# KhutornoyYaroslav/vcm-ts

Hardware: AMD Instinct MI355X
Metric: encoded frames/sec at 1920x1080 GOP-32 (higher is better)
Workload: dtype f32 (fp16x3 split-MFMA, fp32 accumulate)

## Files before the change

### vcm_ts_amd/csrc/conv_mfma.hip

```cpp
#include <hip/hip_runtime.h>
#include <stdint.h>
#include <stdlib.h>
#include <string.h>
#include <type_traits>
#include <vector>

#include "dcvc_hip.h"
#include "kernel_common.h"

namespace {

constexpr int LDK = 20;


struct ConvK {
    const float *seg_ptr[DCVC_MAX_SEG];
    int seg_C[DCVC_MAX_SEG];
    int seg_cs[DCVC_MAX_SEG];
    int nseg;
    int Hin, Win, Hout, Wout;
    int in_act;
    float in_slope;
    const float *wpack;
    const float *bpack;
    int Cout, Cout_pad;
    float *out;
    int out_cs;
    int out_act;
    float out_slope;
    int ps;
    const float *res;
    int res_cs;
    const float *res_gate;
    const float *res2;
    int res2_cs;
    int vec_epi;
    int *status;
    float *chan_partial;
    int ntx;
    int ty0, nty;
    int band_rows;
};

int g_lookahead = 2;

inline long dev_env_long(const char *name, long dflt) {
    const char *dev = getenv("DCVC_DEV");
    if (!dev || strcmp(dev, "1") != 0) return dflt;
    const char *v = getenv(name);
    return v ? atol(v) : dflt;
}


template <int KS, int S, int RPW, int NT, bool SPLIT, bool PAIR = false, bool AHEAD = false>
__global__ __launch_bounds__(256, 2) void conv_mfma(const ConvK a) {
    static_assert(!PAIR || (KS == 7 && S == 1 && SPLIT), "tap pairing is built for the 7x7 split-fp16 layers");
    constexpr int BH = 4 * RPW, BW = 32, BN = 32 * NT;
    constexpr int PH = (BH - 1) * S + KS, PW = (BW - 1) * S + KS, PAD = KS / 2;
    constexpr int T = PAIR ? KS * 4 : KS * KS;
    constexpr int TPS = PAIR ? 4 : (KS == 3 && S == 1) ? 9 : KS;
    constexpr int NST = T / TPS;
    constexpr int EPI_LD = BN + 4;
    constexpr int LDS_MAIN = PH * PW * LDK + TPS * 4 * BN * 4, LDS_EPI = 4 * 32 * EPI_LD, LDS_RED = 4 * BN;
    __shared__ __attribute__((aligned(16))) float lds[LDS_MAIN > LDS_EPI + LDS_RED ? LDS_MAIN : LDS_EPI + LDS_RED];
    float *patch = lds;
    float *wl = lds + PH * PW * LDK;

    const int tid = threadIdx.x, lane = tid & 63, wave = tid >> 6;
    const int nbn = a.Cout_pad / BN;
    const int nb = blockIdx.x % nbn, tx = blockIdx.x / nbn;
    if (tx >= a.ntx) return;
    const int ty = blockIdx.y + a.ty0;
    const int x0 = tx * BW, y0 = ty * BH, n0 = nb * BN, img = blockIdx.z;

    f32x16 acc[RPW][NT];
#pragma unroll
    for (int m = 0; m < RPW; ++m)
#pragma unroll
        for (int n = 0; n < NT; ++n)
#pragma unroll
            for (int r = 0; r < 16; ++r) acc[m][n][r] = 0.f;

    const int a_base = ((wave * RPW * S) * PW + (lane & 31) * S) * LDK + (lane >> 5) * 4;
    const int b_base = ((lane >> 5) * BN + (lane & 31)) * 4;

    constexpr int NP = (PH * PW * 4 + 255) / 256, NW = (TPS * 4 * BN + 255) / 256;
    static_assert(!AHEAD || NST >= 3, "AHEAD: two straight-line steps and a loop over the rest of a chunk");
    f32x4 rp[NP], rw[NW];
    struct Cursor {
        int s, c0, cg, st;
    };
    auto advance = [&](Cursor &k) {
        if (++k.st == NST) {
            k.st = 0;
            ++k.cg;
            k.c0 += MFMA_KC;
            if (k.c0 >= a.seg_C[k.s]) {
                ++k.s;
                k.c0 = 0;
            }
        }
    };
    int poff[NP];
    unsigned inpic = 0;
#pragma unroll
    for (int u = 0; u < NP; ++u) {
        const int i = tid + u * 256;
        const int p = i >> 2;
        const int py = p / PW, px = p - py * PW + (PAIR ? (i & 3) >> 1 : 0);
        const int gy = y0 * S - PAD + py, gx = x0 * S - PAD + px;
        const bool ok = i < PH * PW * 4 && gy >= 0 && gy < a.Hin && gx >= 0 && gx < a.Win;
        poff[u] = ok ? gy * a.Win + gx : 0;
        inpic |= (ok ? 1u : 0u) << u;
    }
    auto load_patch = [&](const Cursor &k) {
        const int C = a.seg_C[k.s], cs = a.seg_cs[k.s];
        const float *sp = a.seg_ptr[k.s] + (size_t)img * a.Hin * a.Win * cs;
        const int c = PAIR ? (tid & 1) * 4 : k.c0 + (tid & 3) * 4;
        const int cc = c < C ? c : 0;
#pragma unroll
        for (int u = 0; u < NP; ++u) rp[u] = *(const f32x4 *)(sp + (size_t)poff[u] * cs + cc);
    };
    auto store_patch = [&](const Cursor &k) {
        const int C = a.seg_C[k.s];
#pragma unroll
        for (int u = 0; u < NP; ++u) {
            const int i = tid + u * 256;
            if (i < PH * PW * 4) {
                const int c = PAIR ? (i & 1) * 4 : k.c0 + (i & 3) * 4;
                f32x4 v = ((inpic >> u) & 1u) && c < C ? rp[u] : (f32x4){0.f, 0.f, 0.f, 0.f};
                if (c + 3 >= C) {
                    if (c + 1 >= C) v[1] = 0.f;
                    if (c + 2 >= C) v[2] = 0.f;
                    v[3] = 0.f;
                }
                if (a.in_act) {
                    v[0] = act(v[0], a.in_slope);
                    v[1] = act(v[1], a.in_slope);
                    v[2] = act(v[2], a.in_slope);
                    v[3] = act(v[3], a.in_slope);
                }
                if (!SPLIT) {
                    *(f32x4 *)&patch[(i >> 2) * LDK + (i & 3) * 4] = v;
                } else {
                    f32x4 sv = v * ACT_SCALE;
#pragma unroll
                    for (int e = 0; e < 4; ++e) sv[e] = __builtin_amdgcn_fmed3f(sv[e], -F16_MAX, F16_MAX);
                    const f16x4 hi = __builtin_convertvector(sv, f16x4);
                    const f16x4 lo = __builtin_convertvector(sv - __builtin_convertvector(hi, f32x4), f16x4);
                    _Float16 *rec = (_Float16 *)&patch[(i >> 2) * LDK];
                    *(f16x4 *)&rec[(i & 3) * 4] = hi;
                    *(f16x4 *)&rec[16 + (i & 3) * 4] = lo;
                }
            }
        }
    };
    constexpr int W_OVER = NW * 256 - TPS * 4 * BN;
    static_assert(!AHEAD || TPS * 4 * BN >= W_OVER, "the doubled float4 must lie inside the slab");
    auto w_slot = [&](const int u) {
        const int i = tid + u * 256;
        return AHEAD && W_OVER > 0 && u == NW - 1 && i >= TPS * 4 * BN ? i - W_OVER : i;
    };
    auto load_w = [&](const Cursor &k) {
        const float *wsrc = a.wpack + ((size_t)(k.cg * T + k.st * TPS) * 4) * a.Cout_pad * 4 + (size_t)n0 * 4;
#pragma unroll
        for (int u = 0; u < NW; ++u) {
            const int i = w_slot(u);
            const int row = i / BN, col = i - row * BN;
            if (AHEAD || i < TPS * 4 * BN) rw[u] = *(const f32x4 *)(wsrc + ((size_t)row * a.Cout_pad + col) * 4);
        }
    };
    auto store_w = [&]() {
#pragma unroll
        for (int u = 0; u < NW; ++u) {
            const int i = w_slot(u);
            if (AHEAD || i < TPS * 4 * BN) *(f32x4 *)&wl[i * 4] = rw[u];
        }
    };
    auto mfma_step = [&](const int st) {
        const int a_st = (TPS == T) ? 0 : st * PW * LDK;
#pragma unroll
        for (int tt = 0; tt < TPS; ++tt) {
            const int ky = (TPS == T) ? tt / KS : 0, kx = PAIR ? 2 * tt : (TPS == T) ? tt % KS : tt;
            if (!SPLIT) {
#pragma unroll
                for (int k2 = 0; k2 < 2; ++k2) {
                    f32x4 af[RPW], bf[NT];
#pragma unroll
                    for (int m = 0; m < RPW; ++m)
                        af[m] = *(const f32x4 *)&patch[a_base + a_st + ((m * S + ky) * PW + kx) * LDK + k2 * 8];
#pragma unroll
                    for (int n = 0; n < NT; ++n)
                        bf[n] = *(const f32x4 *)&wl[b_base + ((tt * 4 + k2 * 2) * BN + n * 32) * 4];
#pragma unroll
                    for (int j = 0; j < 4; ++j)
#pragma unroll
                        for (int m = 0; m < RPW; ++m)
#pragma unroll
                            for (int n = 0; n < NT; ++n)
                                acc[m][n] = __builtin_amdgcn_mfma_f32_32x32x2f32(af[m][j], bf[n][j], acc[m][n], 0, 0, 0);
                }
            } else {
                f16x8 ah[RPW], al[RPW], bh[NT], bl[NT];
#pragma unroll
                for (int m = 0; m < RPW; ++m) {
                    const float *rec = &patch[a_base + a_st + ((m * S + ky) * PW + kx) * LDK];
                    ah[m] = *(const f16x8 *)rec;
                    al[m] = *(const f16x8 *)(rec + 8);
                }
#pragma unroll
                for (int n = 0; n < NT; ++n) {
                    bh[n] = *(const f16x8 *)&wl[b_base + ((tt * 4) * BN + n * 32) * 4];
                    bl[n] = *(const f16x8 *)&wl[b_base + ((tt * 4 + 2) * BN + n * 32) * 4];
                }
#pragma unroll
                for (int m = 0; m < RPW; ++m)
#pragma unroll
                    for (int n = 0; n < NT; ++n) {
                        acc[m][n] = __builtin_amdgcn_mfma_f32_32x32x16_f16(ah[m], bh[n], acc[m][n], 0, 0, 0);
                        acc[m][n] = __builtin_amdgcn_mfma_f32_32x32x16_f16(ah[m], bl[n], acc[m][n], 0, 0, 0);
                        acc[m][n] = __builtin_amdgcn_mfma_f32_32x32x16_f16(al[m], bh[n], acc[m][n], 0, 0, 0);
                    }
            }
        }
    };

    Cursor cur = {0, 0, 0, 0};
    if constexpr (AHEAD) {
        auto chunk = [&](auto more, const Cursor &nc) {
            constexpr bool MORE = decltype(more)::value;
            __syncthreads();
            store_patch(cur);
            store_w();
            __syncthreads();
            advance(cur);
            load_w(cur);
            if (MORE) load_patch(nc);
            mfma_step(0);
            auto row_step = [&](const int st) {
                __syncthreads();
                store_w();
                __syncthreads();
                if (st + 1 < NST) {
                    advance(cur);
                    load_w(cur);
                } else if (MORE) {
                    load_w(nc);
                }
                mfma_step(st);
            };
            row_step(1);
            for (int st = 2; st < NST; ++st) row_step(st);
        };
        load_patch(cur);
        load_w(cur);
        for (;;) {
            Cursor nc = cur;
            nc.st = NST - 1;
            advance(nc);
            if (nc.s >= a.nseg) break;
            chunk(std::true_type{}, nc);
            cur = nc;
        }
        chunk(std::false_type{}, cur);
    } else {
        load_patch(cur);
        load_w(cur);
        while (cur.s < a.nseg) {
            __syncthreads();
            if (cur.st == 0) store_patch(cur);
            store_w();
            __syncthreads();
            Cursor nxt = cur;
            advance(nxt);
            if (nxt.s < a.nseg) {
                if (nxt.st == 0) load_patch(nxt);
                load_w(nxt);
            }
            mfma_step(cur.st);
            cur = nxt;
        }
    }

    const int col = lane & 31, hh = lane >> 5;
    const int Cq = a.Cout >> 2;
    const int Cfin = a.ps ? Cq : a.Cout;
    const int Ho = a.ps ? a.Hout * 2 : a.Hout, Wo = a.ps ? a.Wout * 2 : a.Wout;
    const float inv_scale = SPLIT ? 1.f / (ACT_SCALE * WGT_SCALE) : 1.f;
    float vmax = 0.f;
    if (a.vec_epi) {
        constexpr int LPP = BN / 4, PPI = 64 / LPP, NIT = 32 / PPI;
        float *epi = lds + wave * 32 * EPI_LD;
        const int c4 = (lane % LPP) * 4, pl = lane / LPP;
        const int ch = n0 + c4;
        const bool ch_ok = ch < a.Cout;
        int dy = 0, dx = 0, cf = ch;
        if (a.ps) {
            const int sub = ch / Cq;
            cf = ch - sub * Cq;
            dy = sub >> 1;
            dx = sub & 1;
        }
        f32x4 bias = {0.f, 0.f, 0.f, 0.f}, gate = {1.f, 1.f, 1.f, 1.f};
        if (ch_ok) {
            bias = *(const f32x4 *)&a.bpack[ch];
            if (a.res_gate) gate = *(const f32x4 *)&a.res_gate[(size_t)img * Cfin + cf];
        }
        __syncthreads();
        size_t pix[RPW][NIT];
        bool ok[RPW][NIT];
        f32x4 rv[RPW][NIT], rv2[RPW][NIT];
        f32x4 csum = {0.f, 0.f, 0.f, 0.f};
#pragma unroll
        for (int m = 0; m < RPW; ++m) {
            const int oy = y0 + wave * RPW + m;
#pragma unroll
            for (int it = 0; it < NIT; ++it) {
                const int ox = x0 + it * PPI + pl;
                ok[m][it] = ch_ok && oy < a.Hout && ox < a.Wout;
                pix[m][it] = a.ps ? ((size_t)(img * Ho + 2 * oy + dy) * Wo + 2 * ox + dx) : ((size_t)(img * Ho + oy) * Wo + ox);
                rv[m][it] = (f32x4){0.f, 0.f, 0.f, 0.f};
                rv2[m][it] = (f32x4){0.f, 0.f, 0.f, 0.f};
                if (ok[m][it] && a.res) rv[m][it] = *(const f32x4 *)&a.res[pix[m][it] * a.res_cs + cf];
                if (ok[m][it] && a.res2) rv2[m][it] = *(const f32x4 *)&a.res2[pix[m][it] * a.res2_cs + cf];
            }
        }
#pragma unroll
        for (int m = 0; m < RPW; ++m) {
#pragma unroll
            for (int n = 0; n < NT; ++n)
#pragma unroll
                for (int r = 0; r < 16; ++r)
                    epi[((r & 3) + 8 * (r >> 2) + 4 * hh) * EPI_LD + n * 32 + col] = acc[m][n][r];
            asm volatile("s_waitcnt lgkmcnt(0)" ::: "memory");
#pragma unroll
            for (int it = 0; it < NIT; ++it) {
                f32x4 v = *(const f32x4 *)&epi[(it * PPI + pl) * EPI_LD + c4];
                v = v * inv_scale + bias;
                if (a.out_act == 1) {
                    v[0] = act(v[0], a.out_slope);
                    v[1] = act(v[1], a.out_slope);
                    v[2] = act(v[2], a.out_slope);
                    v[3] = act(v[3], a.out_slope);
                } else if (a.out_act == 2) {
#pragma unroll
                    for (int e = 0; e < 4; ++e) v[e] = fminf(fmaxf(v[e], 0.f), 1.f);
                }
                if (a.out_act == 3) {
#pragma unroll
                    for (int e = 0; e < 4; ++e) {
                        const float mk = rv2[m][it][e] > 0.f ? 1.f : a.out_slope;
                        v[e] = a.res ? __builtin_fmaf(v[e], mk, rv[m][it][e]) : v[e] * mk;
                    }
                } else {
                    if (a.res) {
                        if (a.res_gate) {
#pragma unroll
                            for (int e = 0; e < 4; ++e) v[e] = __builtin_fmaf(rv[m][it][e], gate[e], v[e]);
                        } else {
                            v = v + rv[m][it];
                        }
                    }
                    if (a.res2) v = rv2[m][it] + v;
                }
                if (a.chan_partial && ok[m][it]) csum += v;
                if (a.status && ok[m][it])
                    vmax = fmaxf(vmax, fmaxf(fmaxf(fabsf(v[0]), fabsf(v[1])), fmaxf(fabsf(v[2]), fabsf(v[3]))));
                if (ok[m][it]) *(f32x4 *)&a.out[pix[m][it] * a.out_cs + cf] = v;
            }
            asm volatile("s_waitcnt lgkmcnt(0)" ::: "memory");
        }
        if (a.status && !(vmax <= ACT_LIMIT)) atomicOr(a.status, DCVC_STATUS_ACT_SATURATED);
        if (a.chan_partial) {
#pragma unroll
            for (int off = LPP; off < 64; off <<= 1)
#pragma unroll
                for (int e = 0; e < 4; ++e) csum[e] += __shfl_xor(csum[e], off);
            float *red = lds + LDS_EPI;
            if (lane < LPP) *(f32x4 *)&red[wave * BN + c4] = csum;
            __syncthreads();
            if (tid < BN && n0 + tid < a.Cout_pad) {
                const float s = ((red[tid] + red[BN + tid]) + red[2 * BN + tid]) + red[3 * BN + tid];
                const size_t part = (size_t)img * (a.nty * a.ntx) + (size_t)ty * a.ntx + tx;
                a.chan_partial[part * a.Cout_pad + n0 + tid] = s;
            }
        }
        return;
    }
#pragma unroll
    for (int m = 0; m < RPW; ++m) {
        const int oy = y0 + wave * RPW + m;
        if (oy >= a.Hout) continue;
#pragma unroll
        for (int n = 0; n < NT; ++n) {
            const int ch = n0 + n * 32 + col;
            if (ch >= a.Cout) continue;
            const float bias = a.bpack[ch];
            int dy = 0, dx = 0, cf = ch;
            if (a.ps) {
                const int sub = ch / Cq;
                cf = ch - sub * Cq;
                dy = sub >> 1;
                dx = sub & 1;
            }
            const float gate = a.res_gate ? a.res_gate[(size_t)img * Cfin + cf] : 1.f;
            float rv[16], rv2[16];
#pragma unroll
            for (int r = 0; r < 16; ++r) {
                const int ox = x0 + (r & 3) + 8 * (r >> 2) + 4 * hh;
                const size_t pix = a.ps ? ((size_t)(img * Ho + 2 * oy + dy) * Wo + 2 * ox + dx)
                                        : ((size_t)(img * Ho + oy) * Wo + ox);
                rv[r] = (a.res && ox < a.Wout) ? a.res[pix * a.res_cs + cf] : 0.f;
                rv2[r] = (a.res2 && ox < a.Wout) ? a.res2[pix * a.res2_cs + cf] : 0.f;
            }
#pragma unroll
            for (int r = 0; r < 16; ++r) {
                const int ox = x0 + (r & 3) + 8 * (r >> 2) + 4 * hh;
                if (ox >= a.Wout) continue;
                float v = acc[m][n][r] * inv_scale + bias;
                if (a.out_act == 1) v = act(v, a.out_slope);
                else if (a.out_act == 2) v = fminf(fmaxf(v, 0.f), 1.f);
                const size_t pix = a.ps ? ((size_t)(img * Ho + 2 * oy + dy) * Wo + 2 * ox + dx)
                                        : ((size_t)(img * Ho + oy) * Wo + ox);
                if (a.out_act == 3) {
                    const float mk = rv2[r] > 0.f ? 1.f : a.out_slope;
                    v = a.res ? __builtin_fmaf(v, mk, rv[r]) : v * mk;
                } else {
                    if (a.res) v = a.res_gate ? __builtin_fmaf(rv[r], gate, v) : v + rv[r];
                    if (a.res2) v = rv2[r] + v;
                }
                if (a.status) vmax = fmaxf(vmax, fabsf(v));
                a.out[pix * a.out_cs + cf] = v;
            }
        }
    }
    if (a.status && !(vmax <= ACT_LIMIT)) atomicOr(a.status, DCVC_STATUS_ACT_SATURATED);
}


template <int KS, int S, int RPW, int NT, bool PAIR = false>
int launch(ConvK &k, int N, hipStream_t st, int precision) {
    constexpr int BH = 4 * RPW, BN = 32 * NT;
    k.ntx = (k.Wout + 31) / 32;
    static const bool xcd_pad = dev_env_long("DCVC_XCD_PAD", 0) != 0;
    unsigned gx = (unsigned)(k.ntx * (k.Cout_pad / BN));
    if (xcd_pad && gx >= 8) gx = (gx + 7) & ~7u;
    k.nty = (k.Hout + BH - 1) / BH;
    if (k.ty0 < 0 || k.ty0 >= k.nty) return DCVC_E_ARG;
    const int rows = k.band_rows > 0 ? (k.band_rows < k.nty - k.ty0 ? k.band_rows : k.nty - k.ty0) : k.nty;
    dim3 grid(gx, (unsigned)rows, (unsigned)N);
    constexpr bool HAS_AHEAD = (KS == 3 && S == 2) || KS == 7;
    if constexpr (HAS_AHEAD) {
        if (g_lookahead == 2) {
            if (PAIR)
                hipLaunchKernelGGL((conv_mfma<KS, S, RPW, NT, true, PAIR, true>), grid, dim3(256), 0, st, k);
            else if (precision == DCVC_PREC_FP16X3)
                hipLaunchKernelGGL((conv_mfma<KS, S, RPW, NT, true, false, true>), grid, dim3(256), 0, st, k);
            else
                hipLaunchKernelGGL((conv_mfma<KS, S, RPW, NT, false, false, !(KS == 7 && RPW == 2 && NT == 2)>), grid, dim3(256), 0, st, k);
            RET_LAUNCH();
        }
    }
    if (PAIR)
        hipLaunchKernelGGL((conv_mfma<KS, S, RPW, NT, true, PAIR>), grid, dim3(256), 0, st, k);
    else if (precision == DCVC_PREC_FP16X3)
        hipLaunchKernelGGL((conv_mfma<KS, S, RPW, NT, true>), grid, dim3(256), 0, st, k);
    else
        hipLaunchKernelGGL((conv_mfma<KS, S, RPW, NT, false>), grid, dim3(256), 0, st, k);
    RET_LAUNCH();
}

}

extern "C" int64_t dcvc_conv_pack_size(int32_t Cout, int32_t ks, int32_t nseg, const int32_t *seg_C, int32_t *cout_pad) {
    if (Cout <= 0 || nseg <= 0 || nseg > DCVC_MAX_SEG || (ks != 1 && ks != 3 && ks != 7)) return DCVC_E_ARG;
    int chunks = 0;
    for (int s = 0; s < nseg; ++s) chunks += (seg_C[s] + MFMA_KC - 1) / MFMA_KC;
    const int cp = round_up(Cout, 32);
    if (cout_pad) *cout_pad = cp;
    return (int64_t)chunks * ks * ks * 4 * cp * 4;
}

extern "C" int dcvc_conv_pack_weights(const float *w, const float *b, int32_t Cout, int32_t ks, int32_t nseg,
                                      const int32_t *seg_C, int32_t pixel_shuffle, int32_t precision, float *wpack,
                                      float *bpack) {
    if (precision != DCVC_PREC_FP32 && precision != DCVC_PREC_FP16X3) return DCVC_E_ARG;
    int32_t cp = 0;
    const int64_t total = dcvc_conv_pack_size(Cout, ks, nseg, seg_C, &cp);
    if (total < 0 || (pixel_shuffle && (Cout & 3))) return DCVC_E_ARG;
    const int T = ks * ks;
    int Cin = 0;
    for (int s = 0; s < nseg; ++s) Cin += seg_C[s];
    memset(wpack, 0, (size_t)total * sizeof(float));
    memset(bpack, 0, (size_t)cp * sizeof(float));
    const int Cq = Cout / 4;
    _Float16 *base = (_Float16 *)wpack;
    int cg = 0, cin0 = 0;
    for (int s = 0; s < nseg; ++s) {
        for (int c0 = 0; c0 < seg_C[s]; c0 += MFMA_KC, ++cg) {
            for (int t = 0; t < T; ++t)
                for (int cc = 0; cc < MFMA_KC && c0 + cc < seg_C[s]; ++cc)
                    for (int n = 0; n < Cout; ++n) {
                        const int np = pixel_shuffle ? ps_packed_channel(n, Cq) : n;
                        const float v = w[((size_t)n * Cin + cin0 + c0 + cc) * T + t];
                        if (precision == DCVC_PREC_FP32) {
                            wpack[mfma_wpack_f32(cg, T, t, cc, cp, np)] = v;
                        } else {
                            float sv = v * WGT_SCALE;
                            sv = sv > F16_MAX ? F16_MAX : (sv < -F16_MAX ? -F16_MAX : sv);
                            const SplitF16 p = split_f16(sv);
                            base[mfma_wpack_f16(cg, T, t, cc, cp, np, 0)] = p.hi;
                            base[mfma_wpack_f16(cg, T, t, cc, cp, np, 1)] = p.lo;
                        }
                    }
        }
        cin0 += seg_C[s];
    }
    for (int n = 0; n < Cout; ++n) bpack[pixel_shuffle ? ps_packed_channel(n, Cq) : n] = b ? b[n] : 0.f;
    return DCVC_OK;
}

extern "C" int64_t dcvc_conv_pack_size_paired(int32_t Cout, int32_t Cin, int32_t *cout_pad) {
    if (Cout <= 0 || Cin <= 0 || Cin > 8) return DCVC_E_ARG;
    const int cp = round_up(Cout, 32);
    if (cout_pad) *cout_pad = cp;
    return (int64_t)7 * 4 * 4 * cp * 4;
}

extern "C" int dcvc_conv_pack_weights_paired(const float *w, const float *b, int32_t Cout, int32_t Cin, float *wpack, float *bpack) {
    int32_t cp = 0;
    const int64_t total = dcvc_conv_pack_size_paired(Cout, Cin, &cp);
    if (total < 0 || !w || !wpack || !bpack) return DCVC_E_ARG;
    memset(wpack, 0, (size_t)total * sizeof(float));
    memset(bpack, 0, (size_t)cp * sizeof(float));
    _Float16 *base = (_Float16 *)wpack;
    bool clamped = false;
    for (int ky = 0; ky < 7; ++ky)
        for (int kx = 0; kx < 7; ++kx) {
            const int step = ky * 4 + (kx >> 1), h = kx & 1;
            for (int c = 0; c < Cin; ++c)
                for (int n = 0; n < Cout; ++n) {
                    float sv = w[((size_t)n * Cin + c) * 49 + ky * 7 + kx] * WGT_SCALE;
                    if (!(fabsf(sv) <= F16_MAX)) { clamped = true; sv = sv > 0.f ? F16_MAX : -F16_MAX; }
                    const SplitF16 p = split_f16(sv);
                    base[mfma_wpack_f16(0, 28, step, 8 * h + c, cp, n, 0)] = p.hi;
                    base[mfma_wpack_f16(0, 28, step, 8 * h + c, cp, n, 1)] = p.lo;
                }
        }
    for (int n = 0; n < Cout; ++n) bpack[n] = b ? b[n] : 0.f;
    return clamped ? DCVC_E_RANGE : DCVC_OK;
}

static int tile_rows(int ks, int stride) { return stride == 2 ? 4 : 8; }

extern "C" int32_t dcvc_conv_tile_rows(int32_t ks, int32_t stride) { return tile_rows(ks, stride); }

extern "C" int32_t dcvc_conv_chan_partial_parts(int32_t ks, int32_t stride, int32_t Hout, int32_t Wout) {
    if (Hout <= 0 || Wout <= 0 || (stride != 1 && stride != 2)) return DCVC_E_ARG;
    const int bh = tile_rows(ks, stride);
    return ((Wout + 31) / 32) * ((Hout + bh - 1) / bh);
}

extern "C" int dcvc_conv_set_lookahead(int32_t mode) {
    if (mode != 1 && mode != 2) return DCVC_E_ARG;
    g_lookahead = mode;
    return DCVC_OK;
}

extern "C" int dcvc_conv2d(const dcvc_conv_args *a, void *stream) {
    if (!conv_args_ok(a)) return DCVC_E_ARG;
    if (a->stride != 1 && a->stride != 2) return DCVC_E_ARG;
    if (a->precision != DCVC_PREC_FP32 && a->precision != DCVC_PREC_FP16X3) return DCVC_E_ARG;
    if (a->Cout_pad % 32 || a->Cout > a->Cout_pad || (a->pixel_shuffle && (a->Cout & 3))) return DCVC_E_ARG;
    if (a->out_act < 0 || a->out_act > 3) return DCVC_E_ARG;
    if (a->out_act == 3 && (!a->res2 || a->res_gate || a->chan_partial || a->pixel_shuffle)) return DCVC_E_ARG;
    ConvK k;
    memset(&k, 0, sizeof(k));
    copy_conv_args_full(k, a);
    k.Hin = a->Hin;
    k.Win = a->Win;
    const int pad = a->ks / 2;
    k.Hout = (a->Hin + 2 * pad - a->ks) / a->stride + 1;
    k.Wout = (a->Win + 2 * pad - a->ks) / a->stride + 1;
    k.vec_epi = vec_epilogue_ok(a);
    if (a->chan_partial && (!k.vec_epi || a->pixel_shuffle)) return DCVC_E_ARG;
    hipStream_t st = (hipStream_t)stream;
    const bool wide = (a->Cout_pad % 64) == 0;
    const int key = a->ks * 10 + a->stride;
    if (a->stride == 1 && !a->pair_taps && !a->chan_partial && a->tile_rows <= 0) {
        const long wgs8 = (long)((k.Wout + 31) / 32) * ((k.Hout + 7) / 8) * (a->Cout_pad / (wide ? 64 : 32)) * a->N;
        static const long rows4_below = dev_env_long("DCVC_ROWS4_WGS", 384);
        if (wgs8 < rows4_below) {
            if (a->ks == 3) return wide ? launch<3, 1, 1, 2>(k, a->N, st, a->precision) : launch<3, 1, 1, 1>(k, a->N, st, a->precision);
            if (a->ks == 7) return wide ? launch<7, 1, 1, 2>(k, a->N, st, a->precision) : launch<7, 1, 1, 1>(k, a->N, st, a->precision);
            if (a->ks == 1) return wide ? launch<1, 1, 1, 2>(k, a->N, st, a->precision) : launch<1, 1, 1, 1>(k, a->N, st, a->precision);
        }
    }
    switch (key) {
        case 11: return wide ? launch<1, 1, 2, 2>(k, a->N, st, a->precision) : launch<1, 1, 2, 1>(k, a->N, st, a->precision);
        case 12: return wide ? launch<1, 2, 1, 2>(k, a->N, st, a->precision) : launch<1, 2, 1, 1>(k, a->N, st, a->precision);
        case 31:
            return wide ? launch<3, 1, 2, 2>(k, a->N, st, a->precision) : launch<3, 1, 2, 1>(k, a->N, st, a->precision);
        case 32: return wide ? launch<3, 2, 1, 2>(k, a->N, st, a->precision) : launch<3, 2, 1, 1>(k, a->N, st, a->precision);
        case 71:
            if (a->pair_taps) {
                if (a->nseg != 1 || a->seg[0].C > 8 || a->precision != DCVC_PREC_FP16X3 || a->pixel_shuffle) return DCVC_E_ARG;
                return wide ? launch<7, 1, 2, 2, true>(k, a->N, st, a->precision) : launch<7, 1, 2, 1, true>(k, a->N, st, a->precision);
            }
            return wide ? launch<7, 1, 2, 2>(k, a->N, st, a->precision) : launch<7, 1, 2, 1>(k, a->N, st, a->precision);
        default: return DCVC_E_ARG;
    }
}
```

### vcm_ts_amd/csrc/conv_small.hip

```cpp
#include <hip/hip_runtime.h>
#include <stdint.h>
#include <string.h>

#include "dcvc_hip.h"
#include "kernel_common.h"

namespace {

constexpr int KC = 16;

struct SmallK {
    const float *seg_ptr[DCVC_MAX_SEG];
    int seg_C[DCVC_MAX_SEG];
    int seg_cs[DCVC_MAX_SEG];
    int nseg;
    int H, W;
    int in_act;
    float in_slope;
    const char *wpack;
    const float *bpack;
    int Cout;
    float *out;
    int out_cs, out_act;
    float out_slope;
    const float *res;
    int res_cs;
    int *status;
};

template <int KS>
__global__ __launch_bounds__(256, 3) void conv_small(const SmallK a) {
    constexpr int RPW = 2, BH = 4 * RPW, BW = 32, PAD = KS / 2, PH = BH + KS - 1, PW = BW + KS - 1, T = KS * KS;
    constexpr int TPS = KS, NST = KS;
    constexpr int PATCH_F = PH * PW * 16;
    constexpr int SLAB_F = TPS * 4 * 16 * 4;
    __shared__ __attribute__((aligned(16))) float lds[PATCH_F + SLAB_F];
    char *patch = (char *)lds;
    float *wl = lds + PATCH_F;

    const int tid = threadIdx.x, lane = tid & 63, wave = tid >> 6;
    const int x0 = blockIdx.x * BW, y0 = blockIdx.y * BH, img = blockIdx.z;
    const int pr = lane & 15, g = lane >> 4;

    f32x4 acc[RPW][2];
#pragma unroll
    for (int m = 0; m < RPW; ++m)
#pragma unroll
        for (int hf = 0; hf < 2; ++hf) acc[m][hf] = (f32x4){0.f, 0.f, 0.f, 0.f};

    constexpr int NP = (PH * PW * 4 + 255) / 256, NW = (SLAB_F / 4 + 255) / 256;
    f32x4 rp[NP], rw[NW];
    struct Cursor {
        int s, c0, cg, st;
    };
    auto advance = [&](Cursor &k) {
        if (++k.st == NST) {
            k.st = 0;
            ++k.cg;
            k.c0 += KC;
            if (k.c0 >= a.seg_C[k.s]) {
                ++k.s;
                k.c0 = 0;
            }
        }
    };
    int poff[NP];
    unsigned inpic = 0;
#pragma unroll
    for (int u = 0; u < NP; ++u) {
        const int i = tid + u * 256;
        const int p = i >> 2;
        const int py = p / PW, px = p - py * PW;
        const int gy = y0 - PAD + py, gx = x0 - PAD + px;
        const bool ok = i < PH * PW * 4 && gy >= 0 && gy < a.H && gx >= 0 && gx < a.W;
        poff[u] = ok ? gy * a.W + gx : 0;
        inpic |= (ok ? 1u : 0u) << u;
    }
    auto load_patch = [&](const Cursor &k) {
        const int C = a.seg_C[k.s], cs = a.seg_cs[k.s];
        const float *sp = a.seg_ptr[k.s] + (size_t)img * a.H * a.W * cs;
        const int c = k.c0 + (tid & 3) * 4;
        const int cc = c < C ? c : 0;
#pragma unroll
        for (int u = 0; u < NP; ++u) rp[u] = *(const f32x4 *)(sp + (size_t)poff[u] * cs + cc);
    };
    auto store_patch = [&](const Cursor &k) {
        const int C = a.seg_C[k.s];
#pragma unroll
        for (int u = 0; u < NP; ++u) {
            const int i = tid + u * 256;
            if (i < PH * PW * 4) {
                const int qd = i & 3, p = i >> 2;
                const int c = k.c0 + qd * 4;
                f32x4 v = ((inpic >> u) & 1u) && c < C ? rp[u] : (f32x4){0.f, 0.f, 0.f, 0.f};
                if (c + 3 >= C) {
                    if (c + 1 >= C) v[1] = 0.f;
                    if (c + 2 >= C) v[2] = 0.f;
                    v[3] = 0.f;
                }
                if (a.in_act) {
#pragma unroll
                    for (int e = 0; e < 4; ++e) v[e] = act(v[e], a.in_slope);
                }
                f32x4 sv = v * ACT_SCALE;
#pragma unroll
                for (int e = 0; e < 4; ++e) sv[e] = __builtin_amdgcn_fmed3f(sv[e], -F16_MAX, F16_MAX);
                const f16x4 hi = __builtin_convertvector(sv, f16x4);
                const f16x4 lo = __builtin_convertvector(sv - __builtin_convertvector(hi, f32x4), f16x4);
                const int sw = (p >> 1) & 3, h = qd >> 1;
                char *rec = patch + p * 64 + (qd & 1) * 8;
                *(f16x4 *)(rec + ((h ^ sw) << 4)) = hi;
                *(f16x4 *)(rec + (((2 + h) ^ sw) << 4)) = lo;
            }
        }
    };
    auto load_w = [&](const Cursor &k) {
        const f32x4 *wsrc = (const f32x4 *)(a.wpack + ((size_t)(k.cg * T + k.st * TPS)) * 1024);
#pragma unroll
        for (int u = 0; u < NW; ++u) {
            const int i = tid + u * 256;
            if (i < SLAB_F / 4) rw[u] = wsrc[i];
        }
    };
    auto store_w = [&]() {
#pragma unroll
        for (int u = 0; u < NW; ++u) {
            const int i = tid + u * 256;
            if (i < SLAB_F / 4) *(f32x4 *)&wl[i * 4] = rw[u];
        }
    };

    Cursor cur = {0, 0, 0, 0};
    load_patch(cur);
    load_w(cur);
    const f16x8 zero8 = {0, 0, 0, 0, 0, 0, 0, 0};
    while (cur.s < a.nseg) {
        __syncthreads();
        if (cur.st == 0) store_patch(cur);
        store_w();
        __syncthreads();
        Cursor nxt = cur;
        advance(nxt);
        if (nxt.s < a.nseg) {
            if (nxt.st == 0) load_patch(nxt);
            load_w(nxt);
        }
#pragma unroll
        for (int tt = 0; tt < TPS; ++tt) {
            const f16x8 b1 = *(const f16x8 *)&wl[((tt * 4 + (g & 1)) * 16 + pr) * 4];
            const f16x8 b2 = g < 2 ? *(const f16x8 *)&wl[((tt * 4 + 2 + g) * 16 + pr) * 4] : zero8;
#pragma unroll
            for (int m = 0; m < RPW; ++m)
#pragma unroll
                for (int hf = 0; hf < 2; ++hf) {
                    const int p = (wave * RPW + m + cur.st) * PW + hf * 16 + pr + tt;
                    const f16x8 av = *(const f16x8 *)(patch + p * 64 + ((g ^ ((p >> 1) & 3)) << 4));
                    acc[m][hf] = __builtin_amdgcn_mfma_f32_16x16x32_f16(av, b1, acc[m][hf], 0, 0, 0);
                    acc[m][hf] = __builtin_amdgcn_mfma_f32_16x16x32_f16(av, b2, acc[m][hf], 0, 0, 0);
                }
        }
        cur = nxt;
    }

    const float inv_scale = 1.f / (ACT_SCALE * WGT_SCALE);
    const int ch = pr;
    bool sat = false;
    if (ch < a.Cout) {
        const float bias = a.bpack[ch];
#pragma unroll
        for (int m = 0; m < RPW; ++m) {
            const int oy = y0 + wave * RPW + m;
            if (oy >= a.H) continue;
            float rv[2][4];
#pragma unroll
            for (int hf = 0; hf < 2; ++hf)
#pragma unroll
                for (int j = 0; j < 4; ++j) {
                    const int ox = x0 + hf * 16 + g * 4 + j;
                    rv[hf][j] = (a.res && ox < a.W) ? a.res[((size_t)(img * a.H + oy) * a.W + ox) * a.res_cs + ch] : 0.f;
                }
#pragma unroll
            for (int hf = 0; hf < 2; ++hf)
#pragma unroll
                for (int j = 0; j < 4; ++j) {
                    const int ox = x0 + hf * 16 + g * 4 + j;
                    if (ox >= a.W) continue;
                    float v = acc[m][hf][j] * inv_scale + bias;
                    if (a.out_act == 1) v = act(v, a.out_slope);
                    else if (a.out_act == 2) v = fminf(fmaxf(v, 0.f), 1.f);
                    if (a.res) v += rv[hf][j];
                    if (a.status && !(fabsf(v) <= ACT_LIMIT)) sat = true;
                    a.out[((size_t)(img * a.H + oy) * a.W + ox) * a.out_cs + ch] = v;
                }
        }
    }
    if (sat) atomicOr(a.status, DCVC_STATUS_ACT_SATURATED);
}

}

extern "C" int64_t dcvc_conv_small_pack_bytes(int32_t Cout, int32_t ks, int32_t nseg, const int32_t *seg_C) {
    if (Cout <= 0 || Cout > 16 || nseg <= 0 || nseg > DCVC_MAX_SEG || (ks != 3 && ks != 7)) return DCVC_E_ARG;
    int chunks = 0;
    for (int s = 0; s < nseg; ++s) {
        if (seg_C[s] <= 0) return DCVC_E_ARG;
        chunks += (seg_C[s] + KC - 1) / KC;
    }
    return (int64_t)chunks * ks * ks * 1024;
}

extern "C" int dcvc_conv_small_pack_weights(const float *w, const float *b, int32_t Cout, int32_t ks, int32_t nseg,
                                            const int32_t *seg_C, void *wpack, float *bpack) {
    const int64_t total = dcvc_conv_small_pack_bytes(Cout, ks, nseg, seg_C);
    if (total < 0 || !w || !wpack || !bpack) return DCVC_E_ARG;
    const int T = ks * ks;
    int Cin = 0;
    for (int s = 0; s < nseg; ++s) Cin += seg_C[s];
    memset(wpack, 0, (size_t)total);
    for (int n = 0; n < 16; ++n) bpack[n] = (b && n < Cout) ? b[n] : 0.f;
    _Float16 *base = (_Float16 *)wpack;
    int status = DCVC_OK, cg = 0, cin0 = 0;
    for (int s = 0; s < nseg; ++s) {
        for (int c0 = 0; c0 < seg_C[s]; c0 += KC, ++cg)
            for (int t = 0; t < T; ++t)
                for (int cc = 0; cc < KC && c0 + cc < seg_C[s]; ++cc)
                    for (int n = 0; n < Cout; ++n) {
                        float sv = w[((size_t)n * Cin + cin0 + c0 + cc) * T + t] * WGT_SCALE;
                        if (!(fabsf(sv) <= F16_MAX)) { status = DCVC_E_RANGE; sv = sv > 0.f ? F16_MAX : -F16_MAX; }
                        const SplitF16 p = split_f16(sv);
                        const size_t blk = ((size_t)cg * T + t) * 4;
                        base[((blk + (cc >> 3)) * 16 + n) * 8 + (cc & 7)] = p.hi;
                        base[((blk + 2 + (cc >> 3)) * 16 + n) * 8 + (cc & 7)] = p.lo;
                    }
        cin0 += seg_C[s];
    }
    return status;
}

extern "C" int dcvc_conv2d_small(const dcvc_conv_args *a, void *stream) {
    if (!conv_args_ok(a)) return DCVC_E_ARG;
    if (a->out_act < 0 || a->out_act > 2) return DCVC_E_ARG;
    if (a->tile_rows > 0) return DCVC_E_ARG;
    if (a->Cout <= 0 || a->Cout > 16 || (a->ks != 3 && a->ks != 7) || a->stride != 1 || a->pixel_shuffle || a->res_gate ||
        a->res2 || a->chan_partial || a->precision != DCVC_PREC_FP16X3 || a->N <= 0)
        return DCVC_E_ARG;
    SmallK k;
    memset(&k, 0, sizeof(k));
    copy_conv_args(k, a);
    k.H = a->Hin, k.W = a->Win;
    dim3 grid((unsigned)((a->Win + 31) / 32), (unsigned)((a->Hin + 7) / 8), (unsigned)a->N);
    if (a->ks == 7)
        hipLaunchKernelGGL(conv_small<7>, grid, dim3(256), 0, (hipStream_t)stream, k);
    else
        hipLaunchKernelGGL(conv_small<3>, grid, dim3(256), 0, (hipStream_t)stream, k);
    RET_LAUNCH();
}
```

### vcm_ts_amd/csrc/kernel_common.h

```cpp
#ifndef DCVC_KERNEL_COMMON_H
#define DCVC_KERNEL_COMMON_H

#include <hip/hip_runtime.h>
#include <stdint.h>

#include "dcvc_hip.h"

typedef float f32x16 __attribute__((ext_vector_type(16)));
typedef float f32x4 __attribute__((ext_vector_type(4)));
typedef _Float16 f16x8 __attribute__((ext_vector_type(8)));
typedef _Float16 f16x4 __attribute__((ext_vector_type(4)));

namespace {

#define RET_LAUNCH() return hipGetLastError() == hipSuccess ? DCVC_OK : DCVC_E_LAUNCH
inline unsigned nblk(int64_t n, int b) { return (unsigned)((n + b - 1) / b); }
inline int round_up(int v, int m) { return (v + m - 1) / m * m; }
inline bool aligned16(const void *p, int cs) { return p == nullptr || ((((uintptr_t)p) & 15) == 0 && (cs & 3) == 0); }

constexpr float ACT_SCALE = 8.f;
constexpr float WGT_SCALE = 64.f;
constexpr float F16_MAX = 65504.f;
constexpr float ACT_LIMIT = F16_MAX / ACT_SCALE;

__device__ __forceinline__ float act(float v, float slope) { return v > 0.f ? v : v * slope; }

__device__ __forceinline__ unsigned wave_sum(unsigned v) {
#pragma unroll
    for (int off = 32; off > 0; off >>= 1) v += (unsigned)__shfl_xor((int)v, off);
    return v;
}

__device__ __forceinline__ int32_t scale_index(float s, const float *edges) {
    int lo = 0;
#pragma unroll
    for (int step = 128; step >= 1; step >>= 1)
        if (edges[lo + step - 1] <= s) lo += step;
    return lo;
}

struct SplitF16 {
    _Float16 hi, lo;
};
__host__ __device__ inline SplitF16 split_f16(float sv) {
    const _Float16 hi = (_Float16)sv;
    return {hi, (_Float16)(sv - (float)hi)};
}

__host__ __device__ inline int ps_packed_channel(int n, int Cq) { return (n & 3) * Cq + (n >> 2); }
__host__ __device__ inline int ps_source_channel(int np, int Cq) { return (np % Cq) * 4 + np / Cq; }

constexpr int MFMA_KC = 16;
__host__ __device__ inline size_t mfma_wpack_f32(int cg, int T, int t, int cc, int cp, int np) {
    const int kq = cc >> 2, j = cc & 3;
    return ((((size_t)cg * T + t) * 4 + kq) * cp + np) * 4 + j;
}
__host__ __device__ inline size_t mfma_wpack_f16(int cg, int T, int t, int cc, int cp, int np, int lo) {
    const int h = cc >> 3, jj = cc & 7;
    return ((((size_t)cg * T + t) * 4 + 2 * lo + h) * cp + np) * 8 + jj;
}

inline bool conv_args_ok(const dcvc_conv_args *a) {
    if (!a || a->nseg < 1 || a->nseg > DCVC_MAX_SEG || !a->out || !a->wpack || !a->bpack) return false;
    if (a->N <= 0 || a->Hin <= 0 || a->Win <= 0 || a->Cout <= 0) return false;
    for (int s = 0; s < a->nseg; ++s)
        if (!a->seg[s].ptr || (a->seg[s].cs & 3) || a->seg[s].cs < round_up(a->seg[s].C, 4) || ((uintptr_t)a->seg[s].ptr & 15))
            return false;
    return true;
}

inline bool vec_epilogue_ok(const dcvc_conv_args *a) {
    const int cfin = a->pixel_shuffle ? a->Cout / 4 : a->Cout;
    return cfin % 4 == 0 && aligned16(a->out, a->out_cs) && aligned16(a->res, a->res_cs) && aligned16(a->res2, a->res2_cs) &&
           aligned16(a->res_gate, 0);
}

template <class K>
inline void copy_conv_args(K &k, const dcvc_conv_args *a) {
    for (int s = 0; s < a->nseg; ++s) {
        k.seg_ptr[s] = a->seg[s].ptr;
        k.seg_C[s] = a->seg[s].C;
        k.seg_cs[s] = a->seg[s].cs;
    }
    k.nseg = a->nseg;
    k.in_act = a->in_act;
    k.in_slope = a->in_slope;
    k.wpack = (decltype(k.wpack))a->wpack;
    k.bpack = a->bpack;
    k.Cout = a->Cout;
    k.out = a->out;
    k.out_cs = a->out_cs;
    k.out_act = a->out_act;
    k.out_slope = a->out_slope;
    k.res = a->res;
    k.res_cs = a->res_cs;
    k.status = a->status;
}

template <class K>
inline void copy_conv_args_full(K &k, const dcvc_conv_args *a) {
    copy_conv_args(k, a);
    k.Cout_pad = a->Cout_pad;
    k.ps = a->pixel_shuffle;
    k.res_gate = a->res_gate;
    k.res2 = a->res2;
    k.res2_cs = a->res2_cs;
    k.chan_partial = a->chan_partial;
    k.ty0 = a->tile_rows > 0 ? a->tile_row0 : 0;
    k.band_rows = a->tile_rows > 0 ? a->tile_rows : 0;
}

}

#endif
```

Baseline: 42.76.

## Add lookahead variant of small conv kernel with buffer loads and unrolled stages

```diff
diff --git a/vcm_ts_amd/csrc/conv_mfma.hip b/vcm_ts_amd/csrc/conv_mfma.hip
--- a/vcm_ts_amd/csrc/conv_mfma.hip
+++ b/vcm_ts_amd/csrc/conv_mfma.hip
@@ -42,7 +42,6 @@
     int band_rows;
 };
 
-int g_lookahead = 2;
 
 inline long dev_env_long(const char *name, long dflt) {
     const char *dev = getenv("DCVC_DEV");
@@ -451,7 +450,7 @@
     dim3 grid(gx, (unsigned)rows, (unsigned)N);
     constexpr bool HAS_AHEAD = (KS == 3 && S == 2) || KS == 7;
     if constexpr (HAS_AHEAD) {
-        if (g_lookahead == 2) {
+        if (g_conv_lookahead == 2) {
             if (PAIR)
                 hipLaunchKernelGGL((conv_mfma<KS, S, RPW, NT, true, PAIR, true>), grid, dim3(256), 0, st, k);
             else if (precision == DCVC_PREC_FP16X3)
@@ -561,9 +560,11 @@
     return ((Wout + 31) / 32) * ((Hout + bh - 1) / bh);
 }
 
+int g_conv_lookahead = 2;
+
 extern "C" int dcvc_conv_set_lookahead(int32_t mode) {
     if (mode != 1 && mode != 2) return DCVC_E_ARG;
-    g_lookahead = mode;
+    g_conv_lookahead = mode;
     return DCVC_OK;
 }
 
diff --git a/vcm_ts_amd/csrc/conv_small.hip b/vcm_ts_amd/csrc/conv_small.hip
--- a/vcm_ts_amd/csrc/conv_small.hip
+++ b/vcm_ts_amd/csrc/conv_small.hip
@@ -1,6 +1,8 @@
 #include <hip/hip_runtime.h>
 #include <stdint.h>
 #include <string.h>
+
+#include <type_traits>
 
 #include "dcvc_hip.h"
 #include "kernel_common.h"
@@ -28,7 +30,7 @@
     int *status;
 };
 
-template <int KS>
+template <int KS, bool AHEAD = false>
 __global__ __launch_bounds__(256, 3) void conv_small(const SmallK a) {
     constexpr int RPW = 2, BH = 4 * RPW, BW = 32, PAD = KS / 2, PH = BH + KS - 1, PW = BW + KS - 1, T = KS * KS;
     constexpr int TPS = KS, NST = KS;
@@ -73,18 +75,28 @@
         const int py = p / PW, px = p - py * PW;
         const int gy = y0 - PAD + py, gx = x0 - PAD + px;
         const bool ok = i < PH * PW * 4 && gy >= 0 && gy < a.H && gx >= 0 && gx < a.W;
-        poff[u] = ok ? gy * a.W + gx : 0;
+        poff[u] = ok ? gy * a.W + gx : (AHEAD ? -1 : 0);
         inpic |= (ok ? 1u : 0u) << u;
     }
-    auto load_patch = [&](const Cursor &k) {
+    auto load_patch = [&](const Cursor &k) __attribute__((always_inline)) {
         const int C = a.seg_C[k.s], cs = a.seg_cs[k.s];
         const float *sp = a.seg_ptr[k.s] + (size_t)img * a.H * a.W * cs;
         const int c = k.c0 + (tid & 3) * 4;
         const int cc = c < C ? c : 0;
-#pragma unroll
-        for (int u = 0; u < NP; ++u) rp[u] = *(const f32x4 *)(sp + (size_t)poff[u] * cs + cc);
-    };
-    auto store_patch = [&](const Cursor &k) {
+        if constexpr (AHEAD) {
+            const unsigned img_bytes = (unsigned)(a.H * a.W) * (unsigned)cs * 4u;
+            const __amdgpu_buffer_rsrc_t rs = __builtin_amdgcn_make_buffer_rsrc((void *)sp, 0, (int)img_bytes, 0x00020000);
+#pragma unroll
+            for (int u = 0; u < NP; ++u) {
+                const unsigned off = poff[u] < 0 ? img_bytes : ((unsigned)poff[u] * (unsigned)cs + (unsigned)cc) * 4u;
+                rp[u] = __builtin_bit_cast(f32x4, __builtin_amdgcn_raw_buffer_load_b128(rs, (int)off, 0, 0));
+            }
+        } else {
+#pragma unroll
+            for (int u = 0; u < NP; ++u) rp[u] = *(const f32x4 *)(sp + (size_t)poff[u] * cs + cc);
+        }
+    };
+    auto store_patch = [&](const Cursor &k) __attribute__((always_inline)) {
         const int C = a.seg_C[k.s];
 #pragma unroll
         for (int u = 0; u < NP; ++u) {
@@ -92,7 +104,7 @@
             if (i < PH * PW * 4) {
                 const int qd = i & 3, p = i >> 2;
                 const int c = k.c0 + qd * 4;
-                f32x4 v = ((inpic >> u) & 1u) && c < C ? rp[u] : (f32x4){0.f, 0.f, 0.f, 0.f};
+                f32x4 v = (AHEAD || ((inpic >> u) & 1u)) && c < C ? rp[u] : (f32x4){0.f, 0.f, 0.f, 0.f};
                 if (c + 3 >= C) {
                     if (c + 1 >= C) v[1] = 0.f;
                     if (c + 2 >= C) v[2] = 0.f;
@@ -114,37 +126,36 @@
             }
         }
     };
-    auto load_w = [&](const Cursor &k) {
+    constexpr int W_OVER = NW * 256 - SLAB_F / 4;
+    static_assert(SLAB_F / 4 >= W_OVER, "the doubled float4 must lie inside the row");
+    auto w_slot = [&](const int u) {
+        const int i = tid + u * 256;
+        return AHEAD && W_OVER > 0 && u == NW - 1 && i >= SLAB_F / 4 ? i - W_OVER : i;
+    };
+    auto load_w = [&](const Cursor &k) __attribute__((always_inline)) {
         const f32x4 *wsrc = (const f32x4 *)(a.wpack + ((size_t)(k.cg * T + k.st * TPS)) * 1024);
 #pragma unroll
         for (int u = 0; u < NW; ++u) {
-            const int i = tid + u * 256;
-            if (i < SLAB_F / 4) rw[u] = wsrc[i];
-        }
-    };
-    auto store_w = [&]() {
+            const int i = w_slot(u);
+            if (AHEAD || i < SLAB_F / 4) rw[u] = wsrc[i];
+        }
+    };
+    auto store_w = [&]() __attribute__((always_inline)) {
 #pragma unroll
         for (int u = 0; u < NW; ++u) {
-            const int i = tid + u * 256;
-            if (i < SLAB_F / 4) *(f32x4 *)&wl[i * 4] = rw[u];
-        }
-    };
-
-    Cursor cur = {0, 0, 0, 0};
-    load_patch(cur);
-    load_w(cur);
+            const int i = w_slot(u);
+            if (AHEAD || i < SLAB_F / 4) *(f32x4 *)&wl[i * 4] = rw[u];
+        }
+    };
+
     const f16x8 zero8 = {0, 0, 0, 0, 0, 0, 0, 0};
-    while (cur.s < a.nseg) {
-        __syncthreads();
-        if (cur.st == 0) store_patch(cur);
-        store_w();
-        __syncthreads();
-        Cursor nxt = cur;
-        advance(nxt);
-        if (nxt.s < a.nseg) {
-            if (nxt.st == 0) load_patch(nxt);
-            load_w(nxt);
-        }
+    int abase[8];
+    if constexpr (AHEAD) {
+        const int P0 = wave * RPW * PW + pr;
+#pragma unroll
+        for (int j = 0; j < 8; ++j) abase[j] = P0 * 64 + ((g ^ (((P0 + j) >> 1) & 3)) << 4);
+    }
+    auto mfma_step = [&](const auto st) __attribute__((always_inline)) {
 #pragma unroll
         for (int tt = 0; tt < TPS; ++tt) {
             const f16x8 b1 = *(const f16x8 *)&wl[((tt * 4 + (g & 1)) * 16 + pr) * 4];
@@ -153,19 +164,142 @@
             for (int m = 0; m < RPW; ++m)
 #pragma unroll
                 for (int hf = 0; hf < 2; ++hf) {
-                    const int p = (wave * RPW + m + cur.st) * PW + hf * 16 + pr + tt;
-                    const f16x8 av = *(const f16x8 *)(patch + p * 64 + ((g ^ ((p >> 1) & 3)) << 4));
+                    f16x8 av;
+                    if constexpr (AHEAD) {
+                        const int k = (m + decltype(st)::value) * PW + hf * 16 + tt;
+                        av = *(const f16x8 *)(patch + abase[k & 7] + k * 64);
+                    } else {
+                        const int p = (wave * RPW + m + st) * PW + hf * 16 + pr + tt;
+                        av = *(const f16x8 *)(patch + p * 64 + ((g ^ ((p >> 1) & 3)) << 4));
+                    }
                     acc[m][hf] = __builtin_amdgcn_mfma_f32_16x16x32_f16(av, b1, acc[m][hf], 0, 0, 0);
                     acc[m][hf] = __builtin_amdgcn_mfma_f32_16x16x32_f16(av, b2, acc[m][hf], 0, 0, 0);
                 }
         }
-        cur = nxt;
+    };
+
+    Cursor cur = {0, 0, 0, 0};
+    if constexpr (AHEAD) {
+        auto chunk = [&](auto more, const Cursor &nc) __attribute__((always_inline)) {
+            constexpr bool MORE = decltype(more)::value;
+            __syncthreads();
+            store_patch(cur);
+            store_w();
+            __syncthreads();
+            advance(cur);
+            load_w(cur);
+            if (MORE) load_patch(nc);
+            mfma_step(std::integral_constant<int, 0>{});
+            auto row_step = [&](const auto st) __attribute__((always_inline)) {
+                __syncthreads();
+                store_w();
+                __syncthreads();
+                if (decltype(st)::value + 1 < NST) {
+                    advance(cur);
+                    load_w(cur);
+                } else if (MORE) {
+                    load_w(nc);
+                }
+                mfma_step(st);
+            };
+            static_assert(NST == 3 || NST == 7, "the stages of a chunk are written out");
+            row_step(std::integral_constant<int, 1>{});
+            row_step(std::integral_constant<int, 2>{});
+            if constexpr (NST == 7) {
+                row_step(std::integral_constant<int, 3>{});
+                row_step(std::integral_constant<int, 4>{});
+                row_step(std::integral_constant<int, 5>{});
+                row_step(std::integral_constant<int, 6>{});
+            }
+        };
+        load_patch(cur);
+        load_w(cur);
+        for (;;) {
+            Cursor nc = cur;
+            nc.st = NST - 1;
+            advance(nc);
+            if (nc.s >= a.nseg) break;
+            chunk(std::true_type{}, nc);
+            cur = nc;
+        }
+        chunk(std::false_type{}, cur);
+    } else {
+        load_patch(cur);
+        load_w(cur);
+        while (cur.s < a.nseg) {
+            __syncthreads();
+            if (cur.st == 0) store_patch(cur);
+            store_w();
+            __syncthreads();
+            Cursor nxt = cur;
+            advance(nxt);
+            if (nxt.s < a.nseg) {
+                if (nxt.st == 0) load_patch(nxt);
+                load_w(nxt);
+            }
+            mfma_step(cur.st);
+            cur = nxt;
+        }
     }
 
     const float inv_scale = 1.f / (ACT_SCALE * WGT_SCALE);
     const int ch = pr;
     bool sat = false;
-    if (ch < a.Cout) {
+    if constexpr (AHEAD) {
+        const size_t img_pix = (size_t)img * a.H * a.W;
+        const unsigned out_bytes = ((unsigned)(a.H * a.W - 1) * (unsigned)a.out_cs + (unsigned)a.Cout) * 4u;
+        const __amdgpu_buffer_rsrc_t rs_out =
+            __builtin_amdgcn_make_buffer_rsrc((void *)(a.out + img_pix * a.out_cs), 0, (int)out_bytes, 0x00020000);
+        const float bias = a.bpack[ch];
+        unsigned pix[RPW][2][4];
+#pragma unroll
+        for (int m = 0; m < RPW; ++m)
+#pragma unroll
+            for (int hf = 0; hf < 2; ++hf)
+#pragma unroll
+                for (int j = 0; j < 4; ++j) {
+                    const int oy = y0 + wave * RPW + m, ox = x0 + hf * 16 + g * 4 + j;
+                    const bool ok = (ch < a.Cout) & (oy < a.H) & (ox < a.W);
+                    pix[m][hf][j] = ok ? (unsigned)(oy * a.W + ox) : ~0u;
+                }
+        auto finish = [&](auto with_res) __attribute__((always_inline)) {
+            constexpr bool RES = decltype(with_res)::value;
+            float rv[RPW][2][4];
+            if constexpr (RES) {
+                const unsigned res_bytes = ((unsigned)(a.H * a.W - 1) * (unsigned)a.res_cs + (unsigned)a.Cout) * 4u;
+                const __amdgpu_buffer_rsrc_t rs_res =
+                    __builtin_amdgcn_make_buffer_rsrc((void *)(a.res + img_pix * a.res_cs), 0, (int)res_bytes, 0x00020000);
+#pragma unroll
+                for (int m = 0; m < RPW; ++m)
+#pragma unroll
+                    for (int hf = 0; hf < 2; ++hf)
+#pragma unroll
+                        for (int j = 0; j < 4; ++j) {
+                            const unsigned p = pix[m][hf][j];
+                            const unsigned off = p == ~0u ? res_bytes : (p * (unsigned)a.res_cs + (unsigned)ch) * 4u;
+                            rv[m][hf][j] = __builtin_bit_cast(float, __builtin_amdgcn_raw_buffer_load_b32(rs_res, (int)off, 0, 0));
+                        }
+            }
+#pragma unroll
+            for (int m = 0; m < RPW; ++m)
+#pragma unroll
+                for (int hf = 0; hf < 2; ++hf)
+#pragma unroll
+                    for (int j = 0; j < 4; ++j) {
+                        const unsigned p = pix[m][hf][j];
+                        float v = acc[m][hf][j] * inv_scale + bias;
+                        if (a.out_act == 1) v = act(v, a.out_slope);
+                        else if (a.out_act == 2) v = fminf(fmaxf(v, 0.f), 1.f);
+                        if constexpr (RES) v += rv[m][hf][j];
+                        sat |= (p != ~0u) & !(fabsf(v) <= ACT_LIMIT);
+                        const unsigned off = p == ~0u ? out_bytes : (p * (unsigned)a.out_cs + (unsigned)ch) * 4u;
+                        __builtin_amdgcn_raw_buffer_store_b32(__builtin_bit_cast(int, v), rs_out, (int)off, 0, 0);
+                    }
+        };
+        if (a.res) finish(std::true_type{});
+        else finish(std::false_type{});
+        if (!a.status) sat = false;
+    } else if (ch < a.Cout) {
         const float bias = a.bpack[ch];
 #pragma unroll
         for (int m = 0; m < RPW; ++m) {
@@ -249,9 +383,19 @@
     copy_conv_args(k, a);
     k.H = a->Hin, k.W = a->Win;
     dim3 grid((unsigned)((a->Win + 31) / 32), (unsigned)((a->Hin + 7) / 8), (unsigned)a->N);
-    if (a->ks == 7)
-        hipLaunchKernelGGL(conv_small<7>, grid, dim3(256), 0, (hipStream_t)stream, k);
-    else
-        hipLaunchKernelGGL(conv_small<3>, grid, dim3(256), 0, (hipStream_t)stream, k);
+    auto fits = [&](int cs) { return cs >= 0 && ((unsigned long long)a->Hin * a->Win * cs + 16ull) * 4ull <= 0xfffffff0ull; };
+    bool ahead = g_conv_lookahead == 2 && fits(a->out_cs) && (!a->res || fits(a->res_cs));
+    for (int s = 0; s < a->nseg; ++s) ahead = ahead && fits(a->seg[s].cs);
+    if (a->ks == 7) {
+        if (ahead)
+            hipLaunchKernelGGL((conv_small<7, true>), grid, dim3(256), 0, (hipStream_t)stream, k);
+        else
+            hipLaunchKernelGGL((conv_small<7>), grid, dim3(256), 0, (hipStream_t)stream, k);
+    } else {
+        if (ahead)
+            hipLaunchKernelGGL((conv_small<3, true>), grid, dim3(256), 0, (hipStream_t)stream, k);
+        else
+            hipLaunchKernelGGL((conv_small<3>), grid, dim3(256), 0, (hipStream_t)stream, k);
+    }
     RET_LAUNCH();
 }
diff --git a/vcm_ts_amd/csrc/kernel_common.h b/vcm_ts_amd/csrc/kernel_common.h
--- a/vcm_ts_amd/csrc/kernel_common.h
+++ b/vcm_ts_amd/csrc/kernel_common.h
@@ -10,6 +10,8 @@
 typedef float f32x4 __attribute__((ext_vector_type(4)));
 typedef _Float16 f16x8 __attribute__((ext_vector_type(8)));
 typedef _Float16 f16x4 __attribute__((ext_vector_type(4)));
+
+extern __attribute__((visibility("hidden"))) int g_conv_lookahead;
 
 namespace {
 
```

Result: no change. 43.10, median of 6 (+0.8%).
